# RFD-FHEM/PySignalduino

Hardware: AMD Instinct MI355X
Metric: RF messages/sec demodulated (MU+MS+MC, full protocol bank) (higher is better)
Workload: dtype u8+f64; 1 GPU; mixed MU/MS/MC stream, 1/3 each per rank: MU 256-pulse messages x 129-id MU bank, MS sync+bits x 66-id MS bank (clock x U(0.6,1.4)), MC frames x 12 clockrange ids ('fixed' chain); kind=mixed, corpus=bench, msgs_per_gpu=1000000, batches=3, input_bytes_resident=571611860, parallelism=dp1, grouped=True, streams=one kernel (k_step: MU, then MS, then MC tiles)

## Files before the change

pysignalduino_amd/csrc/sdx_group.hip:

```cpp
#include "sdx_device.h"
#include "sdx_lane.h"

namespace sdx {

SDX_DEV int lanes_below_mask(uint64_t mask) {
  const int l = lane_id();
  return popc64(l ? (mask & ((1ull << l) - 1)) : 0ull);
}
SDX_DEV uint64_t peers8(uint32_t v, bool active) {
  uint64_t peers = ballot(active);
#pragma unroll
  for (int bit = 0; bit < 8; ++bit) {
    const uint64_t bb = ballot(active && ((v >> bit) & 1u));
    peers &= ((v >> bit) & 1u) ? bb : ~bb;
  }
  return peers;
}

constexpr int SIG_PROTOS = 32;
#ifndef SDX_MS_LONG_FIRST
#define SDX_MS_LONG_FIRST 0
#endif
#ifndef SDX_MS_KEY
#define SDX_MS_KEY 0
#endif
template <int KIND>
SDX_DEV void sig_block(const void* __restrict__ bank, const sdx_pulse_batch& b, uint32_t* __restrict__ key,
                       uint32_t* __restrict__ msg_out, sdx_msg_rec* __restrict__ mrec, const int blk) {
  const BankView bv = bank_view(bank);
  const int i = blk * 256 + threadIdx.x;
  const int ntot = b.sel_dev ? b.n_sel : b.n;
  const bool valid = i < ntot;
  const int msg = valid ? (b.sel_dev ? b.sel_dev[i] : i) : 0;
  int npat = valid ? b.npat_dev[msg] : 0;
  npat = npat > SDX_MAXPAT ? SDX_MAXPAT : npat;
  double val[SDX_MAXPAT];
#pragma unroll
  for (int k = 0; k < SDX_MAXPAT; ++k) val[k] = k < npat ? b.pat_val_dev[msg * SDX_MAXPAT + k] : 0.0;
  int kq[SDX_MAXPAT];
  uint32_t sig = 0;
  auto keys_ok = [&](const SpecV& sv) -> bool {
    bool ok = true;
#pragma unroll
    for (int u = 0; u < SDX_MAXUNIQ; ++u) {
      if (u < sv.nu) {
        bool any = false;
#pragma unroll
        for (int j = 0; j < SDX_MAXPAT; ++j) any |= k_in(kq[j], sv.klo[u], sv.khi[u]);
        ok = ok && any;
      }
    }
    return ok;
  };
  if constexpr (KIND == SDX_KIND_MU) {
    float x10[SDX_MAXPAT];
#pragma unroll
    for (int k = 0; k < SDX_MAXPAT; ++k) x10[k] = (float)(val[k] * 10.0);
    const int nr = (int)bv.hdr->n_mu < SIG_PROTOS ? (int)bv.hdr->n_mu : SIG_PROTOS;
    double last = __builtin_nan("");
    for (int r = 0; r < nr; ++r) {
      const sdx_mu_filt* fr = uniform_ptr(bv.mufilt + r);
      const sdx_mu_proto* rec = uniform_ptr(bv.mu + r);
      const uint32_t ff = cld(&fr->flags);
      bool ok = !(ff & 2u) && (ff & 4u);
      if (ok) {
        const double pclk = cld(&fr->clock);
        if (pclk != last) {
          last = pclk;
          const float inv = 1.0f / (float)pclk;
#pragma unroll
          for (int k = 0; k < SDX_MAXPAT; ++k) {
            const float q = x10[k] * inv;
            kq[k] = (k < npat && fabsf(q) < 1.0e8f) ? (int)rintf(q) : SDX_K_NONE;
          }
        }
        const bool full = (ff & 8u) != 0;
        const int k = (ff & 1u) ? 0 : 1;
        const SpecV sv = full ? spec_full(k == 0 ? &rec->start : &rec->one)
                              : spec_compact(&fr->spec[k], k == 0 ? cld(&fr->start_upk) : (uint64_t)cld(&fr->spec[k].upk));
        if (sv.slen) ok = ok && keys_ok(sv);
      }
      sig |= (uint32_t)ok << (31 - r);
    }
  } else {
    const int cp = valid ? b.cp_slot_dev[msg] : -1;
    double clock = 0.0;
#pragma unroll
    for (int k = 0; k < SDX_MAXPAT; ++k)
      if (k == cp) clock = fabs(val[k]);
    const bool gate = valid && b.ms_ok_dev[msg] && cp >= 0 && cp < npat && clock != 0.0;
    const float inv = clock != 0.0 ? (float)(10.0 / clock) : 0.0f;
#pragma unroll
    for (int k = 0; k < SDX_MAXPAT; ++k) {
      const float q = (float)val[k] * inv;
      kq[k] = (gate && k < npat && fabsf(q) < 1.0e8f) ? (int)rintf(q) : SDX_K_NONE;
    }
    const int nr = (int)bv.hdr->n_ms < SIG_PROTOS ? (int)bv.hdr->n_ms : SIG_PROTOS;
    for (int r = 0; r < nr; ++r) {
      const sdx_ms_filt* fr = uniform_ptr(bv.msfilt + r);
      const sdx_ms_proto* rec = uniform_ptr(bv.ms + r);
      const uint32_t ff = cld(&fr->flags);
      bool ok = gate && !(ff & 2u);
      const double pclk = cld(&fr->pclock);
      if (ok && pclk > 0.0) ok = !(fabs(pclk - clock) > clock * 0.3);
      if (ok) {
        const bool full = (ff & 8u) != 0;
        const SpecV sv = full ? spec_full(&rec->key[0]) : spec_compact(&fr->spec[0], cld(&fr->sync_upk));
        if (sv.slen) ok = ok && keys_ok(sv);
      }
      sig |= (uint32_t)ok << (31 - r);
    }
  }
  if (valid && mrec) {
    const int64_t off = b.offsets_dev[msg];
    const int32_t len = b.len_dev ? b.len_dev[msg] : (int32_t)(b.offsets_dev[msg + 1] - off);
    uint32_t id[4] = {0, 0, 0, 0};
#pragma unroll
    for (int k = 0; k < SDX_MAXPAT; ++k) id[k >> 2] |= (uint32_t)b.pat_id_dev[msg * SDX_MAXPAT + k] << (8 * (k & 3));
    const uint32_t w3 = (uint32_t)(valid ? b.npat_dev[msg] : 0) |
                        ((uint32_t)(uint8_t)(KIND == SDX_KIND_MS ? b.cp_slot_dev[msg] : -1) << 8) |
                        ((uint32_t)(KIND == SDX_KIND_MS ? b.ms_ok_dev[msg] : 0) << 16);
    uint4* d = reinterpret_cast<uint4*>(mrec + msg);
    d[0] = make_uint4((uint32_t)off, (uint32_t)((uint64_t)off >> 32), (uint32_t)len, w3);
    d[1] = make_uint4(id[0], id[1], id[2], 0u);
#pragma unroll
    for (int h = 0; h < SDX_MAXPAT / 2; ++h) {
      const uint64_t a = (uint64_t)__double_as_longlong(val[2 * h]), c = (uint64_t)__double_as_longlong(val[2 * h + 1]);
      d[2 + h] = make_uint4((uint32_t)a, (uint32_t)(a >> 32), (uint32_t)c, (uint32_t)(c >> 32));
    }
    d[7] = make_uint4(0u, 0u, 0u, 0u);
  }
  if (valid) {
#if SDX_MS_KEY == 1
    const uint32_t ms_key = ~sig;
#elif SDX_MS_KEY == 2
    const uint32_t ms_key = ((uint32_t)(32 - popc64(sig)) << 26) | (sig >> 6);
#elif SDX_MS_KEY == 3
    const uint32_t ms_key = ((uint32_t)popc64(sig) << 26) | (sig >> 6);
#else
    uint32_t ms_key = sig;
    if (SDX_MS_NARROW) {
      const int64_t o = b.offsets_dev[msg];
      const int len = b.len_dev ? b.len_dev[msg] : (int)(b.offsets_dev[msg + 1] - o);
      ms_key = (((len > 128) != (SDX_MS_LONG_FIRST != 0)) ? 0x80000000u : 0u) | (sig >> 1);
    }
#endif
    key[i] = KIND == SDX_KIND_MU ? ~sig : ms_key;
    msg_out[i] = (uint32_t)msg;
  }
}

template <int KIND>
__global__ __launch_bounds__(256) void k_sig(const void* __restrict__ bank, sdx_pulse_batch b, uint32_t* __restrict__ key,
                                             uint32_t* __restrict__ msg_out, sdx_msg_rec* __restrict__ mrec) {
  sig_block<KIND>(bank, b, key, msg_out, mrec, (int)blockIdx.x);
}

struct SigSide {
  sdx_pulse_batch b;
  uint32_t* key;
  uint32_t* msg;
  sdx_msg_rec* mrec;
};
__global__ __launch_bounds__(256) void k_sig2(const void* __restrict__ bank, SigSide mu, SigSide ms, int g_mu) {
  if ((int)blockIdx.x < g_mu)
    sig_block<SDX_KIND_MU>(bank, mu.b, mu.key, mu.msg, mu.mrec, (int)blockIdx.x);
  else
    sig_block<SDX_KIND_MS>(bank, ms.b, ms.key, ms.msg, ms.mrec, (int)blockIdx.x - g_mu);
}

constexpr int RS_T = 512, RS_ROUNDS = 4, RS_PART = RS_T * RS_ROUNDS;
#ifndef SDX_RS_PASSES
#define SDX_RS_PASSES 4
#endif
#ifndef SDX_RS_PASSES_MS
#define SDX_RS_PASSES_MS SDX_RS_PASSES
#endif
constexpr int RS_PASSES = SDX_RS_PASSES;
constexpr int RS_PASSES_MS = SDX_RS_PASSES_MS;
static_assert(RS_PASSES >= 1 && RS_PASSES <= 4 && RS_PASSES_MS >= 1 && RS_PASSES_MS <= 4, "1..4 radix passes");

SDX_DEV void rs_hist(const uint32_t* __restrict__ key, int n, int np, int d, uint32_t* __restrict__ hist, const int p,
                     uint32_t* c) {
  const int tid = threadIdx.x;
  if (tid < 256) c[tid] = 0;
  __syncthreads();
  for (int r = 0; r < RS_ROUNDS; ++r) {
    const int e = p * RS_PART + r * RS_T + tid;
    const bool valid = e < n;
    const uint32_t dig = valid ? (key[e] >> (8 * d)) & 255u : 0u;
    const uint64_t peers = peers8(dig, valid);
    if (valid && lane_id() == ffs64(peers)) atomicAdd(&c[dig], (uint32_t)popc64(peers));
  }
  __syncthreads();
  if (tid < 256) hist[(size_t)tid * np + p] = c[tid];
}
__global__ __launch_bounds__(RS_T) void k_rs_hist(const uint32_t* __restrict__ key, int n, int np, int d,
                                                  uint32_t* __restrict__ hist) {
  __shared__ uint32_t c[256];
  rs_hist(key, n, np, d, hist, (int)blockIdx.x, c);
}

SDX_DEV void rs_scan_rows(uint32_t* __restrict__ hist, int np, uint32_t* __restrict__ tot, const int blk) {
  const int row = blk * 4 + (threadIdx.x >> 6), lane = threadIdx.x & 63;
  uint32_t* h = hist + (size_t)row * np;
  uint32_t run = 0;
  for (int b0 = 0; b0 < np; b0 += 64) {
    const int x = b0 + lane;
    const uint32_t v = x < np ? h[x] : 0u;
    uint32_t incl = v;
#pragma unroll
    for (int o = 1; o < 64; o <<= 1) {
      const uint32_t y = __shfl_up(incl, o);
      if (lane >= o) incl += y;
    }
    if (x < np) h[x] = run + incl - v;
    run += __shfl(incl, 63);
  }
  if (lane == 0) tot[row] = run;
}
__global__ __launch_bounds__(256) void k_rs_scan_rows(uint32_t* __restrict__ hist, int np, uint32_t* __restrict__ tot) {
  rs_scan_rows(hist, np, tot, (int)blockIdx.x);
}

SDX_DEV void rs_scatter(const uint32_t* __restrict__ kin, const uint32_t* __restrict__ vin, int n, int np, int d,
                        const uint32_t* __restrict__ hist, const uint32_t* __restrict__ tot, uint32_t* __restrict__ kout,
                        uint32_t* __restrict__ vout, const int p, uint32_t* run, uint32_t (*wc)[256]) {
  const int tid = threadIdx.x, wave = tid >> 6;
  const uint32_t t = tid < 256 ? tot[tid] : 0u;
  if (tid < 256) run[tid] = t;
  __syncthreads();
  for (int o = 1; o < 256; o <<= 1) {
    const uint32_t y = (tid < 256 && tid >= o) ? run[tid - o] : 0u;
    __syncthreads();
    if (tid < 256) run[tid] += y;
    __syncthreads();
  }
  if (tid < 256) run[tid] = run[tid] - t + hist[(size_t)tid * np + p];
  for (int r = 0; r < RS_ROUNDS; ++r) {
    const int e = p * RS_PART + r * RS_T + tid;
    const bool valid = e < n;
    const uint32_t k = valid ? kin[e] : 0u;
    const uint32_t v = valid ? vin[e] : 0u;
    const uint32_t dig = (k >> (8 * d)) & 255u;
    for (int x = tid; x < RS_T / 64 * 256; x += RS_T) (&wc[0][0])[x] = 0;
    __syncthreads();
    const uint64_t peers = peers8(dig, valid);
    if (valid && lane_id() == ffs64(peers)) wc[wave][dig] = (uint32_t)popc64(peers);
    __syncthreads();
    if (valid) {
      uint32_t pos = run[dig] + (uint32_t)lanes_below_mask(peers);
      for (int w = 0; w < wave; ++w) pos += wc[w][dig];
      kout[pos] = k;
      vout[pos] = v;
    }
    __syncthreads();
    if (tid < 256) {
      uint32_t add = 0;
#pragma unroll
      for (int w = 0; w < RS_T / 64; ++w) add += wc[w][tid];
      run[tid] += add;
    }
    __syncthreads();
  }
}
__global__ __launch_bounds__(RS_T) void k_rs_scatter(const uint32_t* __restrict__ kin, const uint32_t* __restrict__ vin,
                                                     int n, int np, int d, const uint32_t* __restrict__ hist,
                                                     const uint32_t* __restrict__ tot, uint32_t* __restrict__ kout,
                                                     uint32_t* __restrict__ vout) {
  __shared__ uint32_t run[256];
  __shared__ uint32_t wc[RS_T / 64][256];
  rs_scatter(kin, vin, n, np, d, hist, tot, kout, vout, (int)blockIdx.x, run, wc);
}

struct RsPass {
  const uint32_t* kin;
  const uint32_t* vin;
  uint32_t* kout;
  uint32_t* vout;
  uint32_t* hist;
  uint32_t* tot;
  int n, np;
};
__global__ __launch_bounds__(RS_T) void k_rs_hist2(RsPass a, RsPass b, int d) {
  __shared__ uint32_t c[256];
  const bool second = (int)blockIdx.x >= a.np;
  const RsPass& x = second ? b : a;
  rs_hist(x.kin, x.n, x.np, d, x.hist, second ? (int)blockIdx.x - a.np : (int)blockIdx.x, c);
}
__global__ __launch_bounds__(256) void k_rs_scan_rows2(RsPass a, RsPass b) {
  const bool second = blockIdx.x >= 256 / 4;
  const RsPass& x = second ? b : a;
  rs_scan_rows(x.hist, x.np, x.tot, (int)blockIdx.x - (second ? 256 / 4 : 0));
}
__global__ __launch_bounds__(RS_T) void k_rs_scatter2(RsPass a, RsPass b, int d) {
  __shared__ uint32_t run[256];
  __shared__ uint32_t wc[RS_T / 64][256];
  const bool second = (int)blockIdx.x >= a.np;
  const RsPass& x = second ? b : a;
  rs_scatter(x.kin, x.vin, x.n, x.np, d, x.hist, x.tot, x.kout, x.vout,
             second ? (int)blockIdx.x - a.np : (int)blockIdx.x, run, wc);
}

constexpr size_t align256(size_t x) { return (x + 255) & ~(size_t)255; }

size_t group_bytes(int n) {
  if (n <= 0) return 0;
  const size_t np = (size_t)(n + RS_PART - 1) / RS_PART;
  return 4 * align256(4 * (size_t)n) + align256(4 * 256 * np) + align256(4 * 256);
}

bool group_messages(const void* bank_dev, int kind, const sdx_pulse_batch& b, int32_t* order, sdx_msg_rec* mrec,
                    uint8_t* work, size_t bytes, hipStream_t st) {
  const int n = b.sel_dev ? b.n_sel : b.n;
  const size_t need = group_bytes(n);
  if (!need || bytes < need) return false;
  const int np = (n + RS_PART - 1) / RS_PART;
  const size_t a = align256(4 * (size_t)n);
  uint32_t* k0 = reinterpret_cast<uint32_t*>(work);
  uint32_t* v0 = reinterpret_cast<uint32_t*>(work + a);
  uint32_t* k1 = reinterpret_cast<uint32_t*>(work + 2 * a);
  uint32_t* v1 = reinterpret_cast<uint32_t*>(work + 3 * a);
  uint32_t* hist = reinterpret_cast<uint32_t*>(work + 4 * a);
  uint32_t* tot = reinterpret_cast<uint32_t*>(work + 4 * a + align256(4 * 256 * (size_t)np));
  const int grid = (n + 255) / 256;
  if (kind == SDX_KIND_MU)
    hipLaunchKernelGGL((k_sig<SDX_KIND_MU>), dim3(grid), dim3(256), 0, st, bank_dev, b, k0, v0, mrec);
  else
    hipLaunchKernelGGL((k_sig<SDX_KIND_MS>), dim3(grid), dim3(256), 0, st, bank_dev, b, k0, v0, mrec);
  const int passes = kind == SDX_KIND_MU ? RS_PASSES : RS_PASSES_MS;
  for (int pi = 0; pi < passes; ++pi) {
    const int d = 4 - passes + pi;
    const bool even = (pi & 1) == 0;
    uint32_t* kin = even ? k0 : k1;
    uint32_t* vout = pi == passes - 1 ? reinterpret_cast<uint32_t*>(order) : (even ? v1 : v0);
    hipLaunchKernelGGL(k_rs_hist, dim3(np), dim3(RS_T), 0, st, kin, n, np, d, hist);
    hipLaunchKernelGGL(k_rs_scan_rows, dim3(256 / 4), dim3(256), 0, st, hist, np, tot);
    hipLaunchKernelGGL(k_rs_scatter, dim3(np), dim3(RS_T), 0, st, kin, even ? v0 : v1, n, np, d, hist, tot,
                       even ? k1 : k0, vout);
  }
  return hipGetLastError() == hipSuccess;
}

bool group_messages2(const void* bank_dev, const sdx_pulse_batch& bmu, int32_t* omu, sdx_msg_rec* rmu, uint8_t* wmu,
                     size_t cmu, const sdx_pulse_batch& bms, int32_t* oms, sdx_msg_rec* rms, uint8_t* wms, size_t cms,
                     hipStream_t st) {
  static_assert(RS_PASSES == RS_PASSES_MS, "one pass count for both sorts");
  const int nmu = bmu.sel_dev ? bmu.n_sel : bmu.n, nms = bms.sel_dev ? bms.n_sel : bms.n;
  if (nmu <= 0 || nms <= 0 || cmu < group_bytes(nmu) || cms < group_bytes(nms)) return false;
  struct Side {
    uint32_t *k0, *v0, *k1, *v1, *hist, *tot;
    int n, np;
  };
  auto side = [](uint8_t* work, int n) {
    Side x;
    const size_t a = align256(4 * (size_t)n);
    x.n = n;
    x.np = (n + RS_PART - 1) / RS_PART;
    x.k0 = reinterpret_cast<uint32_t*>(work);
    x.v0 = reinterpret_cast<uint32_t*>(work + a);
    x.k1 = reinterpret_cast<uint32_t*>(work + 2 * a);
    x.v1 = reinterpret_cast<uint32_t*>(work + 3 * a);
    x.hist = reinterpret_cast<uint32_t*>(work + 4 * a);
    x.tot = reinterpret_cast<uint32_t*>(work + 4 * a + align256(4 * 256 * (size_t)x.np));
    return x;
  };
  const Side A = side(wmu, nmu), B = side(wms, nms);
  const int gmu = (nmu + 255) / 256, gms = (nms + 255) / 256;
  hipLaunchKernelGGL(k_sig2, dim3(gmu + gms), dim3(256), 0, st, bank_dev, SigSide{bmu, A.k0, A.v0, rmu},
                     SigSide{bms, B.k0, B.v0, rms}, gmu);
  for (int pi = 0; pi < RS_PASSES; ++pi) {
    const int d = 4 - RS_PASSES + pi;
    const bool even = (pi & 1) == 0;
    const bool last = pi == RS_PASSES - 1;
    auto pass = [&](const Side& x, int32_t* order) {
      return RsPass{even ? x.k0 : x.k1, even ? x.v0 : x.v1, even ? x.k1 : x.k0,
                    last ? reinterpret_cast<uint32_t*>(order) : (even ? x.v1 : x.v0), x.hist, x.tot, x.n, x.np};
    };
    const RsPass pa = pass(A, omu), pb = pass(B, oms);
    hipLaunchKernelGGL(k_rs_hist2, dim3(A.np + B.np), dim3(RS_T), 0, st, pa, pb, d);
    hipLaunchKernelGGL(k_rs_scan_rows2, dim3(2 * (256 / 4)), dim3(256), 0, st, pa, pb);
    hipLaunchKernelGGL(k_rs_scatter2, dim3(A.np + B.np), dim3(RS_T), 0, st, pa, pb, d);
  }
  return hipGetLastError() == hipSuccess;
}

}
```

Measured before the change: 699.1 million msgs/s.

## Restructure radix sort to per-wave contiguous runs with register-held keys

The radix-sort histogram and scatter kernels now give each wave a contiguous run of 64*KPT keys held in registers. Digits are counted into a per-wave shared row with plain lane atomics instead of peer ballots. The scatter loads keys once, computes per-wave digit offsets with a single block barrier, and replaces the 256-wide shared-memory scan of digit totals with a one-wave shuffle scan. Scatter positions come from a per-group atomic on the wave's row, which removes most of the per-round __syncthreads. The risk is extra register pressure and shared atomic contention, and element order within a partition changes to wave-major. Stability is kept because waves take increasing offsets.

```diff
diff --git a/pysignalduino_amd/csrc/sdx_group.hip b/pysignalduino_amd/csrc/sdx_group.hip
--- a/pysignalduino_amd/csrc/sdx_group.hip
+++ b/pysignalduino_amd/csrc/sdx_group.hip
@@ -16,7 +16,6 @@
   }
   return peers;
 }
-
 constexpr int SIG_PROTOS = 32;
 #ifndef SDX_MS_LONG_FIRST
 #define SDX_MS_LONG_FIRST 0
@@ -169,7 +168,13 @@
     sig_block<SDX_KIND_MS>(bank, ms.b, ms.key, ms.msg, ms.mrec, (int)blockIdx.x - g_mu);
 }
 
-constexpr int RS_T = 512, RS_ROUNDS = 4, RS_PART = RS_T * RS_ROUNDS;
+#ifndef SDX_RS_KPT
+#define SDX_RS_KPT 4
+#endif
+#ifndef SDX_RS_COUNT_LANE
+#define SDX_RS_COUNT_LANE 1
+#endif
+constexpr int RS_T = 512, RS_W = RS_T / 64, RS_KPT = SDX_RS_KPT, RS_PART = RS_T * RS_KPT;
 #ifndef SDX_RS_PASSES
 #define SDX_RS_PASSES 4
 #endif
@@ -180,25 +185,56 @@
 constexpr int RS_PASSES_MS = SDX_RS_PASSES_MS;
 static_assert(RS_PASSES >= 1 && RS_PASSES <= 4 && RS_PASSES_MS >= 1 && RS_PASSES_MS <= 4, "1..4 radix passes");
 
+SDX_DEV void rs_wave_sync() {
+  __builtin_amdgcn_fence(__ATOMIC_SEQ_CST, "wavefront");
+  __builtin_amdgcn_wave_barrier();
+}
+SDX_DEV int rs_run_base(int p) { return (p * RS_W + (int)(threadIdx.x >> 6)) * (64 * RS_KPT); }
+SDX_DEV void rs_load(const uint32_t* __restrict__ in, int base, int n, uint32_t (&x)[RS_KPT]) {
+  const int lane = lane_id();
+#pragma unroll
+  for (int j = 0; j < RS_KPT; ++j) {
+    const int e = base + 64 * j + lane;
+    x[j] = e < n ? in[e] : 0u;
+  }
+}
+SDX_DEV void rs_count(const uint32_t (&k)[RS_KPT], int base, int n, int d, uint32_t* row) {
+  const int lane = lane_id();
+#pragma unroll
+  for (int i = 0; i < 256 / 64; ++i) row[lane + 64 * i] = 0;
+  rs_wave_sync();
+#pragma unroll
+  for (int j = 0; j < RS_KPT; ++j) {
+    if (base + 64 * j >= n) break;
+    const bool valid = base + 64 * j + lane < n;
+    const uint32_t dig = (k[j] >> (8 * d)) & 255u;
+#if SDX_RS_COUNT_LANE
+    if (valid) atomicAdd(&row[dig], 1u);
+#else
+    const uint64_t peers = peers8(dig, valid);
+    if (valid && lane == ffs64(peers)) atomicAdd(&row[dig], (uint32_t)popc64(peers));
+#endif
+  }
+}
+
 SDX_DEV void rs_hist(const uint32_t* __restrict__ key, int n, int np, int d, uint32_t* __restrict__ hist, const int p,
-                     uint32_t* c) {
-  const int tid = threadIdx.x;
-  if (tid < 256) c[tid] = 0;
+                     uint32_t (*wc)[256]) {
+  const int tid = threadIdx.x, base = rs_run_base(p);
+  uint32_t k[RS_KPT];
+  rs_load(key, base, n, k);
+  rs_count(k, base, n, d, wc[tid >> 6]);
   __syncthreads();
-  for (int r = 0; r < RS_ROUNDS; ++r) {
-    const int e = p * RS_PART + r * RS_T + tid;
-    const bool valid = e < n;
-    const uint32_t dig = valid ? (key[e] >> (8 * d)) & 255u : 0u;
-    const uint64_t peers = peers8(dig, valid);
-    if (valid && lane_id() == ffs64(peers)) atomicAdd(&c[dig], (uint32_t)popc64(peers));
-  }
-  __syncthreads();
-  if (tid < 256) hist[(size_t)tid * np + p] = c[tid];
+  if (tid < 256) {
+    uint32_t c = 0;
+#pragma unroll
+    for (int w = 0; w < RS_W; ++w) c += wc[w][tid];
+    hist[(size_t)tid * np + p] = c;
+  }
 }
 __global__ __launch_bounds__(RS_T) void k_rs_hist(const uint32_t* __restrict__ key, int n, int np, int d,
                                                   uint32_t* __restrict__ hist) {
-  __shared__ uint32_t c[256];
-  rs_hist(key, n, np, d, hist, (int)blockIdx.x, c);
+  __shared__ uint32_t wc[RS_W][256];
+  rs_hist(key, n, np, d, hist, (int)blockIdx.x, wc);
 }
 
 SDX_DEV void rs_scan_rows(uint32_t* __restrict__ hist, int np, uint32_t* __restrict__ tot, const int blk) {
@@ -225,52 +261,61 @@
 
 SDX_DEV void rs_scatter(const uint32_t* __restrict__ kin, const uint32_t* __restrict__ vin, int n, int np, int d,
                         const uint32_t* __restrict__ hist, const uint32_t* __restrict__ tot, uint32_t* __restrict__ kout,
-                        uint32_t* __restrict__ vout, const int p, uint32_t* run, uint32_t (*wc)[256]) {
-  const int tid = threadIdx.x, wave = tid >> 6;
-  const uint32_t t = tid < 256 ? tot[tid] : 0u;
-  if (tid < 256) run[tid] = t;
+                        uint32_t* __restrict__ vout, const int p, uint32_t* dbase, uint32_t (*wc)[256]) {
+  const int tid = threadIdx.x, wave = tid >> 6, lane = lane_id(), base = rs_run_base(p);
+  uint32_t k[RS_KPT], v[RS_KPT];
+  rs_load(kin, base, n, k);
+  rs_load(vin, base, n, v);
+  const uint32_t off = tid < 256 ? hist[(size_t)tid * np + p] : 0u;
+  if (wave == 0) {
+    const uint4 t = make_uint4(tot[4 * lane], tot[4 * lane + 1], tot[4 * lane + 2], tot[4 * lane + 3]);
+    const uint32_t sum = t.x + t.y + t.z + t.w;
+    uint32_t incl = sum;
+#pragma unroll
+    for (int o = 1; o < 64; o <<= 1) {
+      const uint32_t y = __shfl_up(incl, o);
+      if (lane >= o) incl += y;
+    }
+    const uint32_t e0 = incl - sum;
+    reinterpret_cast<uint4*>(dbase)[lane] = make_uint4(e0, e0 + t.x, e0 + t.x + t.y, e0 + t.x + t.y + t.z);
+  }
+  uint32_t* row = wc[wave];
+  rs_count(k, base, n, d, row);
   __syncthreads();
-  for (int o = 1; o < 256; o <<= 1) {
-    const uint32_t y = (tid < 256 && tid >= o) ? run[tid - o] : 0u;
-    __syncthreads();
-    if (tid < 256) run[tid] += y;
-    __syncthreads();
-  }
-  if (tid < 256) run[tid] = run[tid] - t + hist[(size_t)tid * np + p];
-  for (int r = 0; r < RS_ROUNDS; ++r) {
-    const int e = p * RS_PART + r * RS_T + tid;
-    const bool valid = e < n;
-    const uint32_t k = valid ? kin[e] : 0u;
-    const uint32_t v = valid ? vin[e] : 0u;
-    const uint32_t dig = (k >> (8 * d)) & 255u;
-    for (int x = tid; x < RS_T / 64 * 256; x += RS_T) (&wc[0][0])[x] = 0;
-    __syncthreads();
+  if (tid < 256) {
+    uint32_t acc = dbase[tid] + off;
+#pragma unroll
+    for (int w = 0; w < RS_W; ++w) {
+      const uint32_t c = wc[w][tid];
+      wc[w][tid] = acc;
+      acc += c;
+    }
+  }
+  __syncthreads();
+#pragma unroll
+  for (int j = 0; j < RS_KPT; ++j) {
+    if (base + 64 * j >= n) break;
+    const bool valid = base + 64 * j + lane < n;
+    const uint32_t dig = (k[j] >> (8 * d)) & 255u;
     const uint64_t peers = peers8(dig, valid);
-    if (valid && lane_id() == ffs64(peers)) wc[wave][dig] = (uint32_t)popc64(peers);
-    __syncthreads();
+    const int lead = valid ? ffs64(peers) : lane;
+    uint32_t at = 0;
+    if (valid && lane == lead) at = atomicAdd(&row[dig], (uint32_t)popc64(peers));
+    at = __shfl(at, lead);
     if (valid) {
-      uint32_t pos = run[dig] + (uint32_t)lanes_below_mask(peers);
-      for (int w = 0; w < wave; ++w) pos += wc[w][dig];
-      kout[pos] = k;
-      vout[pos] = v;
-    }
-    __syncthreads();
-    if (tid < 256) {
-      uint32_t add = 0;
-#pragma unroll
-      for (int w = 0; w < RS_T / 64; ++w) add += wc[w][tid];
-      run[tid] += add;
-    }
-    __syncthreads();
+      const uint32_t pos = at + (uint32_t)lanes_below_mask(peers);
+      kout[pos] = k[j];
+      vout[pos] = v[j];
+    }
   }
 }
 __global__ __launch_bounds__(RS_T) void k_rs_scatter(const uint32_t* __restrict__ kin, const uint32_t* __restrict__ vin,
                                                      int n, int np, int d, const uint32_t* __restrict__ hist,
                                                      const uint32_t* __restrict__ tot, uint32_t* __restrict__ kout,
                                                      uint32_t* __restrict__ vout) {
-  __shared__ uint32_t run[256];
-  __shared__ uint32_t wc[RS_T / 64][256];
-  rs_scatter(kin, vin, n, np, d, hist, tot, kout, vout, (int)blockIdx.x, run, wc);
+  __shared__ __attribute__((aligned(16))) uint32_t dbase[256];
+  __shared__ uint32_t wc[RS_W][256];
+  rs_scatter(kin, vin, n, np, d, hist, tot, kout, vout, (int)blockIdx.x, dbase, wc);
 }
 
 struct RsPass {
@@ -283,10 +328,10 @@
   int n, np;
 };
 __global__ __launch_bounds__(RS_T) void k_rs_hist2(RsPass a, RsPass b, int d) {
-  __shared__ uint32_t c[256];
+  __shared__ uint32_t wc[RS_W][256];
   const bool second = (int)blockIdx.x >= a.np;
   const RsPass& x = second ? b : a;
-  rs_hist(x.kin, x.n, x.np, d, x.hist, second ? (int)blockIdx.x - a.np : (int)blockIdx.x, c);
+  rs_hist(x.kin, x.n, x.np, d, x.hist, second ? (int)blockIdx.x - a.np : (int)blockIdx.x, wc);
 }
 __global__ __launch_bounds__(256) void k_rs_scan_rows2(RsPass a, RsPass b) {
   const bool second = blockIdx.x >= 256 / 4;
@@ -294,12 +339,12 @@
   rs_scan_rows(x.hist, x.np, x.tot, (int)blockIdx.x - (second ? 256 / 4 : 0));
 }
 __global__ __launch_bounds__(RS_T) void k_rs_scatter2(RsPass a, RsPass b, int d) {
-  __shared__ uint32_t run[256];
-  __shared__ uint32_t wc[RS_T / 64][256];
+  __shared__ __attribute__((aligned(16))) uint32_t dbase[256];
+  __shared__ uint32_t wc[RS_W][256];
   const bool second = (int)blockIdx.x >= a.np;
   const RsPass& x = second ? b : a;
   rs_scatter(x.kin, x.vin, x.n, x.np, d, x.hist, x.tot, x.kout, x.vout,
-             second ? (int)blockIdx.x - a.np : (int)blockIdx.x, run, wc);
+             second ? (int)blockIdx.x - a.np : (int)blockIdx.x, dbase, wc);
 }
 
 constexpr size_t align256(size_t x) { return (x + 255) & ~(size_t)255; }
```

Measured after the change: 705.0 million msgs/s, median of 6. No clear change (+0.9%).
